# Nostrademous/dotaclient

Hardware: AMD Instinct MI355X
Metric: PPO optimizer samples/sec (whole node) + actor steps/sec, 1v1-mid LSTM policy (higher is better)
Workload: dtype fp32

## Files before the change

### dotaclient_amd/ops/csrc/gemm_tn.hip

```cpp
#include "common.h"
#include <cstdlib>

namespace {

using dca::bf16x8;
using dca::f32x4;
typedef short bf16x4v __attribute__((ext_vector_type(4)));

constexpr int BM = 128, BN = 128, BK = 64;
constexpr int kThreads = 256;
constexpr int kTileBytes = BK * 128 * 2;

__device__ __forceinline__ int lds_off(int row, int ch) {
  return 256 * row + 16 * (ch ^ (((row & 3) << 2) | ((row >> 2) & 3)));
}

__device__ __forceinline__ __amdgpu_buffer_rsrc_t uniform_rsrc(const void* p, long long bytes) {
  const unsigned long long a = (unsigned long long)p;
  const unsigned lo = __builtin_amdgcn_readfirstlane((unsigned)a);
  const unsigned hi = __builtin_amdgcn_readfirstlane((unsigned)(a >> 32));
  const int nb = (int)(bytes < 0 ? 0 : (bytes > 0x7fff0000LL ? 0x7fff0000LL : bytes));
  return __builtin_amdgcn_make_buffer_rsrc((void*)(((unsigned long long)hi << 32) | lo), (short)0,
                                           __builtin_amdgcn_readfirstlane(nb), 0x00020000);
}
constexpr int kOob = 0x7fff8000;

__device__ __forceinline__ uint4 bload16(__amdgpu_buffer_rsrc_t r, int off) {
  return __builtin_bit_cast(uint4, __builtin_amdgcn_raw_buffer_load_b128(r, off, 0, 0));
}

struct Args {
  const void* A; int lda;
  const void* B; int ldb;
  const void* B0; int split;
  float* C; int ldc;
  const int* perm;
  float* slab;
  float* colsum;
  int M, N, K, kc, splits, tiles_n, accumulate;
  int xcd_remap;
};

struct Rsrc {
  __amdgpu_buffer_rsrc_t A, B, B0;
};

__device__ __forceinline__ Rsrc make_rsrc(const Args& a, int es) {
  Rsrc r;
  r.A = uniform_rsrc(a.A, ((long long)(a.K - 1) * a.lda + a.M) * es);
  r.B = uniform_rsrc(a.B, a.K > a.split ? ((long long)(a.K - a.split - 1) * a.ldb + a.N) * es : 0);
  r.B0 = uniform_rsrc(a.B0 ? a.B0 : a.B, a.split > 0 ? ((long long)(a.split - 1) * a.ldb + a.N) * es : 0);
  return r;
}

template <bool WITH_B0>
__device__ __forceinline__ void load_stage(const Args& a, const Rsrc& R, int kbase, int kend, int m_base, int n_base,
                                           uint4 (&ra)[4], uint4 (&rb)[4]) {
  const int t = threadIdx.x, ch = t & 15;
  const int m = m_base + ch * 8, n = n_base + ch * 8;
#pragma unroll
  for (int i = 0; i < 4; ++i) {
    const int k = kbase + (t >> 4) + 16 * i;
    const bool kin = k < kend;
    ra[i] = bload16(R.A, kin && m < a.M ? (k * a.lda + m) * 2 : kOob);
    rb[i] = bload16(R.B, kin && n < a.N && k >= a.split ? ((k - a.split) * a.ldb + n) * 2 : kOob);
  }
  if (WITH_B0 && kbase < a.split) {
#pragma unroll
    for (int i = 0; i < 4; ++i) {
      const int k = kbase + (t >> 4) + 16 * i;
      const uint4 v = bload16(R.B0, k < kend && n < a.N && k < a.split ? (k * a.ldb + n) * 2 : kOob);
      rb[i] = make_uint4(rb[i].x | v.x, rb[i].y | v.y, rb[i].z | v.z, rb[i].w | v.w);
    }
  }
}

__device__ __forceinline__ void store_stage(char* As, char* Bs, const uint4 (&ra)[4], const uint4 (&rb)[4]) {
  const int t = threadIdx.x, ch = t & 15;
#pragma unroll
  for (int i = 0; i < 4; ++i) {
    const int r = (t >> 4) + 16 * i;
    *reinterpret_cast<uint4*>(As + lds_off(r, ch)) = ra[i];
    *reinterpret_cast<uint4*>(Bs + lds_off(r, ch)) = rb[i];
  }
}

__device__ __forceinline__ void colsum_acc(float (&cs)[8], const uint4 (&ra)[4]) {
#pragma unroll
  for (int i = 0; i < 4; ++i) {
    const unsigned w[4] = {ra[i].x, ra[i].y, ra[i].z, ra[i].w};
#pragma unroll
    for (int j = 0; j < 4; ++j) {
      cs[2 * j] += __uint_as_float(w[j] << 16);
      cs[2 * j + 1] += __uint_as_float(w[j] & 0xffff0000u);
    }
  }
}

struct F32Stage {
  float4 a[2][2], b[2][2];
};

template <bool WITH_B0>
__device__ __forceinline__ void load_stage_f32(const Args& a, const Rsrc& R, int kbase, int kend, int m_base,
                                               int n_base, F32Stage& r) {
  const int t = threadIdx.x, ch = t & 15;
  const int m = m_base + ch * 8, n = n_base + ch * 8;
#pragma unroll
  for (int i = 0; i < 2; ++i) {
    const int k = kbase + (t >> 4) + 16 * i;
    const bool kin = k < kend;
    const int oa = kin && m < a.M ? (k * a.lda + m) * 4 : kOob;
    const int ob = kin && n < a.N && k >= a.split ? ((k - a.split) * a.ldb + n) * 4 : kOob;
    r.a[i][0] = __builtin_bit_cast(float4, bload16(R.A, oa));
    r.a[i][1] = __builtin_bit_cast(float4, bload16(R.A, oa + 16));
    r.b[i][0] = __builtin_bit_cast(float4, bload16(R.B, ob));
    r.b[i][1] = __builtin_bit_cast(float4, bload16(R.B, ob + 16));
  }
  if (WITH_B0 && kbase < a.split) {
#pragma unroll
    for (int i = 0; i < 2; ++i) {
      const int k = kbase + (t >> 4) + 16 * i;
      const int o0 = k < kend && n < a.N && k < a.split ? (k * a.ldb + n) * 4 : kOob;
      const float4 p = __builtin_bit_cast(float4, bload16(R.B0, o0));
      const float4 q = __builtin_bit_cast(float4, bload16(R.B0, o0 + 16));
      r.b[i][0] = make_float4(r.b[i][0].x + p.x, r.b[i][0].y + p.y, r.b[i][0].z + p.z, r.b[i][0].w + p.w);
      r.b[i][1] = make_float4(r.b[i][1].x + q.x, r.b[i][1].y + q.y, r.b[i][1].z + q.z, r.b[i][1].w + q.w);
    }
  }
}

__device__ __forceinline__ unsigned pack_bf2(float x, float y) {
  return (unsigned)(unsigned short)dca::f2bf(x) | ((unsigned)(unsigned short)dca::f2bf(y) << 16);
}

__device__ __forceinline__ void split8(const float4& p, const float4& q, uint4& hi, uint4& lo) {
  const float v[8] = {p.x, p.y, p.z, p.w, q.x, q.y, q.z, q.w};
  float l[8];
#pragma unroll
  for (int j = 0; j < 8; ++j) l[j] = v[j] - dca::bf2f(dca::f2bf(v[j]));
  hi = make_uint4(pack_bf2(v[0], v[1]), pack_bf2(v[2], v[3]), pack_bf2(v[4], v[5]), pack_bf2(v[6], v[7]));
  lo = make_uint4(pack_bf2(l[0], l[1]), pack_bf2(l[2], l[3]), pack_bf2(l[4], l[5]), pack_bf2(l[6], l[7]));
}

constexpr int kImgF32 = 32 * 256;
__device__ __forceinline__ void store_stage_f32(char* S, const F32Stage& r) {
  const int t = threadIdx.x, ch = t & 15;
#pragma unroll
  for (int i = 0; i < 2; ++i) {
    const int row = (t >> 4) + 16 * i;
    uint4 hi, lo;
    split8(r.a[i][0], r.a[i][1], hi, lo);
    *reinterpret_cast<uint4*>(S + lds_off(row, ch)) = hi;
    *reinterpret_cast<uint4*>(S + kImgF32 + lds_off(row, ch)) = lo;
    split8(r.b[i][0], r.b[i][1], hi, lo);
    *reinterpret_cast<uint4*>(S + 2 * kImgF32 + lds_off(row, ch)) = hi;
    *reinterpret_cast<uint4*>(S + 3 * kImgF32 + lds_off(row, ch)) = lo;
  }
}

__device__ __forceinline__ void colsum_acc_f32(float (&cs)[8], const F32Stage& r) {
#pragma unroll
  for (int i = 0; i < 2; ++i) {
    cs[0] += r.a[i][0].x; cs[1] += r.a[i][0].y; cs[2] += r.a[i][0].z; cs[3] += r.a[i][0].w;
    cs[4] += r.a[i][1].x; cs[5] += r.a[i][1].y; cs[6] += r.a[i][1].z; cs[7] += r.a[i][1].w;
  }
}

__device__ __forceinline__ bf16x8 frag_tr(const char* img, int k0, int c0) {
  const int l = threadIdx.x & 63, g = l >> 4, i = l & 15, q = i >> 2, p = i & 3;
  const int ch = (c0 >> 3) + (p >> 1);
  const int row0 = k0 + 8 * g + q;
  typedef __attribute__((address_space(3))) bf16x4v lds_v4;
  const bf16x4v lo = __builtin_amdgcn_ds_read_tr16_b64_v4i16(
      (lds_v4*)(img + lds_off(row0, ch) + 8 * (p & 1)));
  const bf16x4v hi = __builtin_amdgcn_ds_read_tr16_b64_v4i16(
      (lds_v4*)(img + lds_off(row0 + 4, ch) + 8 * (p & 1)));
  bf16x8 f;
  f[0] = lo[0]; f[1] = lo[1]; f[2] = lo[2]; f[3] = lo[3];
  f[4] = hi[0]; f[5] = hi[1]; f[6] = hi[2]; f[7] = hi[3];
  return f;
}

__device__ __forceinline__ void tile_split(const Args& a, int& tile, int& split) {
  const int tiles = ((a.M + BM - 1) / BM) * a.tiles_n;
  const int n = gridDim.x, orig = blockIdx.x;
  const int q = n >> 3, r = n & 7, x = orig & 7;
  const int id = a.xcd_remap ? (x < r ? x * (q + 1) : r * (q + 1) + (x - r) * q) + (orig >> 3) : orig;
  tile = id % tiles;
  split = id / tiles;
}

template <bool F32>
__global__ __launch_bounds__(kThreads) void gemm_tn_kernel(Args a) {
  extern __shared__ __attribute__((aligned(16))) char smem[];
  constexpr int BKx = F32 ? 32 : BK;
#define AS(b) (smem + (b) * kTileBytes)
#define BS(b) (smem + (2 + (b)) * kTileBytes)
#define SF(b) (smem + (b) * 4 * kImgF32)
  int tile, split;
  tile_split(a, tile, split);
  const int tm = tile / a.tiles_n, tn = tile % a.tiles_n;
  const int m_base = tm * BM, n_base = tn * BN;
  const int k_lo = split * a.kc, k_hi = min(a.K, k_lo + a.kc);
  const int w = threadIdx.x >> 6, wm = w & 1, wn = w >> 1;

  f32x4 acc[4][4];
#pragma unroll
  for (int i = 0; i < 4; ++i)
#pragma unroll
    for (int j = 0; j < 4; ++j) acc[i][j] = f32x4{0.f, 0.f, 0.f, 0.f};

  uint4 ra[4], rb[4];
  F32Stage rf;
  float cs[8] = {0.f, 0.f, 0.f, 0.f, 0.f, 0.f, 0.f, 0.f};
  const bool do_cs = a.colsum != nullptr && tn == 0;
  int buf = 0;
  const Rsrc R = make_rsrc(a, F32 ? 4 : 2);
  if (k_lo < k_hi) {
    if constexpr (F32) {
      load_stage_f32<true>(a, R, k_lo, k_hi, m_base, n_base, rf);
      store_stage_f32(SF(0), rf);
      if (do_cs) colsum_acc_f32(cs, rf);
    } else {
      load_stage<true>(a, R, k_lo, k_hi, m_base, n_base, ra, rb);
      store_stage(AS(0), BS(0), ra, rb);
      if (do_cs) colsum_acc(cs, ra);
    }
  }
  __syncthreads();
  for (int kb = k_lo; kb < k_hi; kb += BKx) {
    const bool more = kb + BKx < k_hi;
    if constexpr (F32) {
      if (more) load_stage_f32<false>(a, R, kb + BKx, k_hi, m_base, n_base, rf);
      const char* S = SF(buf);
      bf16x8 fah[4], fal[4], fbh[4], fbl[4];
#pragma unroll
      for (int i = 0; i < 4; ++i) {
        fah[i] = frag_tr(S, 0, wm * 64 + i * 16);
        fal[i] = frag_tr(S + kImgF32, 0, wm * 64 + i * 16);
      }
#pragma unroll
      for (int j = 0; j < 4; ++j) {
        fbh[j] = frag_tr(S + 2 * kImgF32, 0, wn * 64 + j * 16);
        fbl[j] = frag_tr(S + 3 * kImgF32, 0, wn * 64 + j * 16);
      }
#pragma unroll
      for (int i = 0; i < 4; ++i)
#pragma unroll
        for (int j = 0; j < 4; ++j) acc[i][j] = __builtin_amdgcn_mfma_f32_16x16x32_bf16(fal[i], fbh[j], acc[i][j], 0, 0, 0);
#pragma unroll
      for (int i = 0; i < 4; ++i)
#pragma unroll
        for (int j = 0; j < 4; ++j) acc[i][j] = __builtin_amdgcn_mfma_f32_16x16x32_bf16(fah[i], fbl[j], acc[i][j], 0, 0, 0);
#pragma unroll
      for (int i = 0; i < 4; ++i)
#pragma unroll
        for (int j = 0; j < 4; ++j) acc[i][j] = __builtin_amdgcn_mfma_f32_16x16x32_bf16(fah[i], fbh[j], acc[i][j], 0, 0, 0);
      if (more) {
        store_stage_f32(SF(buf ^ 1), rf);
        if (do_cs) colsum_acc_f32(cs, rf);
      }
    } else {
      if (more) load_stage<false>(a, R, kb + BK, k_hi, m_base, n_base, ra, rb);
#pragma unroll
      for (int ks = 0; ks < BK / 32; ++ks) {
        bf16x8 fa[4], fb[4];
#pragma unroll
        for (int i = 0; i < 4; ++i) fa[i] = frag_tr(AS(buf), ks * 32, wm * 64 + i * 16);
#pragma unroll
        for (int j = 0; j < 4; ++j) fb[j] = frag_tr(BS(buf), ks * 32, wn * 64 + j * 16);
#pragma unroll
        for (int i = 0; i < 4; ++i)
#pragma unroll
          for (int j = 0; j < 4; ++j)
            acc[i][j] = __builtin_amdgcn_mfma_f32_16x16x32_bf16(fa[i], fb[j], acc[i][j], 0, 0, 0);
      }
      if (more) {
        store_stage(AS(buf ^ 1), BS(buf ^ 1), ra, rb);
        if (do_cs) colsum_acc(cs, ra);
      }
    }
    __syncthreads();
    buf ^= 1;
  }
  if (do_cs) {
    float* red = reinterpret_cast<float*>(smem);
    const int t = threadIdx.x, ch = t & 15, rg = t >> 4;
#pragma unroll
    for (int j = 0; j < 8; ++j) red[rg * 128 + ch * 8 + j] = cs[j];
    __syncthreads();
    if (t < 128) {
      float v = 0.f;
      for (int g = 0; g < 16; ++g) v += red[g * 128 + t];
      const int m = m_base + t;
      if (m < a.M) {
        if (a.splits == 1) {
          float* cp = a.colsum + (a.perm ? a.perm[m] : m);
          *cp = a.accumulate ? *cp + v : v;
        } else {
          a.slab[(size_t)a.splits * a.M * a.N + (size_t)split * a.M + m] = v;
        }
      }
    }
  }

  const int l = threadIdx.x & 63;
  if (a.splits == 1) {
#pragma unroll
    for (int i = 0; i < 4; ++i)
#pragma unroll
      for (int e = 0; e < 4; ++e) {
        const int m = m_base + wm * 64 + 16 * i + 4 * (l >> 4) + e;
        if (m >= a.M) continue;
        float* crow = a.C + (size_t)(a.perm ? a.perm[m] : m) * a.ldc;
#pragma unroll
        for (int j = 0; j < 4; ++j) {
          const int n = n_base + wn * 64 + 16 * j + (l & 15);
          if (n < a.N) crow[n] = a.accumulate ? crow[n] + acc[i][j][e] : acc[i][j][e];
        }
      }
    return;
  }
  float* slab = a.slab + (size_t)split * a.M * a.N;
#pragma unroll
  for (int i = 0; i < 4; ++i)
#pragma unroll
    for (int e = 0; e < 4; ++e) {
      const int m = m_base + wm * 64 + 16 * i + 4 * (l >> 4) + e;
      if (m >= a.M) continue;
#pragma unroll
      for (int j = 0; j < 4; ++j) {
        const int n = n_base + wn * 64 + 16 * j + (l & 15);
        if (n < a.N) slab[(size_t)m * a.N + n] = acc[i][j][e];
      }
    }
#undef AS
#undef BS
#undef SF
}

constexpr int kXP = 144;
constexpr int kXImg = 32 * kXP * 4;

struct XStage {
  float4 a[4], b[4];
};

template <bool WITH_B0>
__device__ __forceinline__ void load_stage_x(const Args& a, const Rsrc& R, int kbase, int kend, int m_base, int n_base,
                                             XStage& r) {
  const int t = threadIdx.x, c4 = 4 * (t & 31);
  const int m = m_base + c4, n = n_base + c4;
#pragma unroll
  for (int i = 0; i < 4; ++i) {
    const int k = kbase + (t >> 5) + 8 * i;
    const bool kin = k < kend;
    r.a[i] = __builtin_bit_cast(float4, bload16(R.A, kin && m < a.M ? (k * a.lda + m) * 4 : kOob));
    r.b[i] = __builtin_bit_cast(float4, bload16(R.B, kin && n < a.N && k >= a.split ? ((k - a.split) * a.ldb + n) * 4
                                                                                    : kOob));
  }
  if (WITH_B0 && kbase < a.split) {
#pragma unroll
    for (int i = 0; i < 4; ++i) {
      const int k = kbase + (t >> 5) + 8 * i;
      const float4 p = __builtin_bit_cast(float4, bload16(R.B0, k < kend && n < a.N && k < a.split ? (k * a.ldb + n) * 4
                                                                                                  : kOob));
      r.b[i] = make_float4(r.b[i].x + p.x, r.b[i].y + p.y, r.b[i].z + p.z, r.b[i].w + p.w);
    }
  }
}

__device__ __forceinline__ void store_stage_x(char* S, const XStage& r) {
  const int t = threadIdx.x, c4 = 4 * (t & 31);
#pragma unroll
  for (int i = 0; i < 4; ++i) {
    const int row = (t >> 5) + 8 * i;
    *reinterpret_cast<float4*>(S + (row * kXP + c4) * 4) = r.a[i];
    *reinterpret_cast<float4*>(S + kXImg + (row * kXP + c4) * 4) = r.b[i];
  }
}

__device__ __forceinline__ void kahan_add(float& s, float& c, float v) {
  const float y = v - c, t = s + y;
  c = (t - s) - y;
  s = t;
}
__device__ __forceinline__ void add_slab_colsum(float (&cs)[4], float (&cc)[4], const XStage& st) {
  kahan_add(cs[0], cc[0], (st.a[0].x + st.a[1].x) + (st.a[2].x + st.a[3].x));
  kahan_add(cs[1], cc[1], (st.a[0].y + st.a[1].y) + (st.a[2].y + st.a[3].y));
  kahan_add(cs[2], cc[2], (st.a[0].z + st.a[1].z) + (st.a[2].z + st.a[3].z));
  kahan_add(cs[3], cc[3], (st.a[0].w + st.a[1].w) + (st.a[2].w + st.a[3].w));
}

__global__ __launch_bounds__(kThreads, 2) void gemm_tn_exact_kernel(Args a) {
  __shared__ __attribute__((aligned(16))) char smem[4 * kXImg];
  int tile, split;
  tile_split(a, tile, split);
  const int tm = tile / a.tiles_n, tn = tile % a.tiles_n;
  const int m_base = tm * BM, n_base = tn * BN;
  const int k_lo = split * a.kc, k_hi = min(a.K, k_lo + a.kc);
  const int w = threadIdx.x >> 6, wm = w & 1, wn = w >> 1, l = threadIdx.x & 63;
  const int fr = l >> 4, fc = l & 15;

  f32x4 acc[4][4];
#pragma unroll
  for (int i = 0; i < 4; ++i)
#pragma unroll
    for (int j = 0; j < 4; ++j) acc[i][j] = f32x4{0.f, 0.f, 0.f, 0.f};
  float cs[4] = {0.f, 0.f, 0.f, 0.f}, cc[4] = {0.f, 0.f, 0.f, 0.f};
  const bool do_cs = a.colsum != nullptr && tn == 0;
  const Rsrc R = make_rsrc(a, 4);
  XStage st;
  int buf = 0;
  if (k_lo < k_hi) {
    load_stage_x<true>(a, R, k_lo, k_hi, m_base, n_base, st);
    store_stage_x(smem, st);
    if (do_cs) add_slab_colsum(cs, cc, st);
  }
  __syncthreads();
  for (int kb = k_lo; kb < k_hi; kb += 32) {
    const bool more = kb + 32 < k_hi;
    if (more) load_stage_x<false>(a, R, kb + 32, k_hi, m_base, n_base, st);
    const float* As = reinterpret_cast<const float*>(smem + buf * 2 * kXImg);
    const float* Bs = As + kXImg / 4;
    f32x4 part[4][4];
#pragma unroll
    for (int i = 0; i < 4; ++i)
#pragma unroll
      for (int j = 0; j < 4; ++j) part[i][j] = f32x4{0.f, 0.f, 0.f, 0.f};
#pragma unroll
    for (int c = 0; c < 8; ++c) {
      const int row = 4 * c + fr;
      float fa[4], fb[4];
#pragma unroll
      for (int i = 0; i < 4; ++i) fa[i] = As[row * kXP + wm * 64 + 16 * i + fc];
#pragma unroll
      for (int j = 0; j < 4; ++j) fb[j] = Bs[row * kXP + wn * 64 + 16 * j + fc];
#pragma unroll
      for (int i = 0; i < 4; ++i)
#pragma unroll
        for (int j = 0; j < 4; ++j) part[i][j] = __builtin_amdgcn_mfma_f32_16x16x4f32(fa[i], fb[j], part[i][j], 0, 0, 0);
    }
#pragma unroll
    for (int i = 0; i < 4; ++i)
#pragma unroll
      for (int j = 0; j < 4; ++j) acc[i][j] += part[i][j];
    if (more) {
      store_stage_x(smem + (buf ^ 1) * 2 * kXImg, st);
      if (do_cs) add_slab_colsum(cs, cc, st);
    }
    __syncthreads();
    buf ^= 1;
  }
  if (do_cs) {
    float* red = reinterpret_cast<float*>(smem);
    const int t = threadIdx.x, c4 = 4 * (t & 31), rg = t >> 5;
#pragma unroll
    for (int j = 0; j < 4; ++j) red[rg * 128 + c4 + j] = cs[j];
    __syncthreads();
    if (t < 128) {
      float v = 0.f;
      for (int g = 0; g < 8; ++g) v += red[g * 128 + t];
      const int m = m_base + t;
      if (m < a.M) {
        if (a.splits == 1) {
          float* cp = a.colsum + (a.perm ? a.perm[m] : m);
          *cp = a.accumulate ? *cp + v : v;
        } else {
          a.slab[(size_t)a.splits * a.M * a.N + (size_t)split * a.M + m] = v;
        }
      }
    }
  }
  float* slab = a.slab + (size_t)split * a.M * a.N;
#pragma unroll
  for (int i = 0; i < 4; ++i)
#pragma unroll
    for (int e = 0; e < 4; ++e) {
      const int m = m_base + wm * 64 + 16 * i + 4 * fr + e;
      if (m >= a.M) continue;
      if (a.splits == 1) {
        float* crow = a.C + (size_t)(a.perm ? a.perm[m] : m) * a.ldc;
#pragma unroll
        for (int j = 0; j < 4; ++j) {
          const int n = n_base + wn * 64 + 16 * j + fc;
          if (n < a.N) crow[n] = a.accumulate ? crow[n] + acc[i][j][e] : acc[i][j][e];
        }
      } else {
#pragma unroll
        for (int j = 0; j < 4; ++j) {
          const int n = n_base + wn * 64 + 16 * j + fc;
          if (n < a.N) slab[(size_t)m * a.N + n] = acc[i][j][e];
        }
      }
    }
}

__global__ __launch_bounds__(256) void gemm_tn_reduce(const float* __restrict__ slab, int splits, int M, int N,
                                                      float* __restrict__ C, int ldc, const int* __restrict__ perm,
                                                      int accumulate, float* __restrict__ colsum, int lp) {
  const int P = 1 << lp, OPB = 256 >> lp;
  const int n4 = N >> 2;
  const size_t plane4 = (size_t)M * N / 4;
  const int ph = threadIdx.x >> (8 - lp), oi = threadIdx.x & (OPB - 1);
  __shared__ f32x4 red[256];
  const int nout = M * n4;
  for (int base = blockIdx.x * OPB; base < nout; base += gridDim.x * OPB) {
    const int idx = base + oi;
    f32x4 s = {0.f, 0.f, 0.f, 0.f};
    if (idx < nout) {
      const int m = idx / n4, n = (idx % n4) * 4;
      const f32x4* src = reinterpret_cast<const f32x4*>(slab + (size_t)m * N + n);
      int sp = ph;
      for (; sp + 3 * P < splits; sp += 4 * P) {
        const f32x4 v0 = __builtin_nontemporal_load(src + (size_t)(sp + 0 * P) * plane4);
        const f32x4 v1 = __builtin_nontemporal_load(src + (size_t)(sp + 1 * P) * plane4);
        const f32x4 v2 = __builtin_nontemporal_load(src + (size_t)(sp + 2 * P) * plane4);
        const f32x4 v3 = __builtin_nontemporal_load(src + (size_t)(sp + 3 * P) * plane4);
        s += v0;
        s += v1;
        s += v2;
        s += v3;
      }
      for (; sp < splits; sp += P) s += __builtin_nontemporal_load(src + (size_t)sp * plane4);
    }
    if (P > 1) {
      red[threadIdx.x] = s;
      __syncthreads();
    }
    if (ph == 0 && idx < nout) {
      for (int k = 1; k < P; ++k) s += red[k * OPB + oi];
      const int m = idx / n4, n = (idx % n4) * 4;
      float* cp = C + (size_t)(perm ? perm[m] : m) * ldc + n;
      if (accumulate) {
        s[0] += cp[0]; s[1] += cp[1]; s[2] += cp[2]; s[3] += cp[3];
      }
      cp[0] = s[0]; cp[1] = s[1]; cp[2] = s[2]; cp[3] = s[3];
    }
    if (P > 1) __syncthreads();
  }
  if (colsum != nullptr) {
    const float* cs = slab + (size_t)splits * plane4 * 4;
    __shared__ float cred[256];
    for (int base = blockIdx.x * OPB; base < M; base += gridDim.x * OPB) {
      const int m = base + oi;
      float v = 0.f;
      if (m < M) {
        int sp = ph;
        for (; sp + 3 * P < splits; sp += 4 * P) {
          const float v0 = cs[(size_t)(sp + 0 * P) * M + m], v1 = cs[(size_t)(sp + 1 * P) * M + m];
          const float v2 = cs[(size_t)(sp + 2 * P) * M + m], v3 = cs[(size_t)(sp + 3 * P) * M + m];
          v += v0;
          v += v1;
          v += v2;
          v += v3;
        }
        for (; sp < splits; sp += P) v += cs[(size_t)sp * M + m];
      }
      cred[threadIdx.x] = v;
      __syncthreads();
      if (ph == 0 && m < M) {
        for (int k = 1; k < P; ++k) v += cred[k * OPB + oi];
        float* cp = colsum + (perm ? perm[m] : m);
        *cp = accumulate ? *cp + v : v;
      }
      __syncthreads();
    }
  }
}

}

extern "C" void dca_gemm_tn_plan(int M, int N, int K, int* splits, int* kc, int* tiles, int f32) {
  const int bk = f32 ? 32 : BK;
  const int tm = (M + BM - 1) / BM, tn = (N + BN - 1) / BN;
  const int t = tm * tn;
  const int target = f32 == 2 ? 512 : 384;
  int s = t >= target ? 1 : target / t;
  const int kmax = (K + bk - 1) / bk;
  if (s > kmax) s = kmax;
  if (s < 1) s = 1;
  int c = (K + s - 1) / s;
  c = (c + bk - 1) / bk * bk;
  s = (K + c - 1) / c;
  *splits = s;
  *kc = c;
  *tiles = t;
}

extern "C" hipError_t dca_gemm_tn(const void* A, int lda, const void* B, int ldb, const void* B0, int split_rows,
                                  float* C, int ldc, const int* perm, int accumulate, int M, int N, int K, float* slab,
                                  float* colsum, hipStream_t st, int f32) {
  if (B0 && split_rows > (f32 ? 32 : BK)) return hipErrorInvalidValue;
  int splits, kc, tiles;
  dca_gemm_tn_plan(M, N, K, &splits, &kc, &tiles, f32);
  static const int xcd_remap = [] { const char* e = getenv("DCA_GEMM_XCD"); return (e && e[0] == '0') ? 0 : 1; }();
  Args a{A, lda, B, ldb, B0 ? B0 : B, B0 ? split_rows : 0, C, ldc, perm, slab, colsum, M, N, K, kc, splits,
         (N + BN - 1) / BN, accumulate, xcd_remap};
  const dim3 grid(tiles * splits);
  if (f32 == 2) hipLaunchKernelGGL(gemm_tn_exact_kernel, grid, dim3(kThreads), 0, st, a);
  else if (f32) hipLaunchKernelGGL(gemm_tn_kernel<true>, grid, dim3(kThreads), 8 * kImgF32, st, a);
  else hipLaunchKernelGGL(gemm_tn_kernel<false>, grid, dim3(kThreads), 4 * kTileBytes, st, a);
  DCA_CHECK_LAUNCH();
  if (splits > 1) {
    int lp = 0;
    while (lp < 4 && (2 << lp) <= splits) ++lp;
    const int n = M * (N / 4), opb = 256 >> lp;
    int blocks = (n + opb - 1) / opb;
    if (blocks > 4096) blocks = 4096;
    hipLaunchKernelGGL(gemm_tn_reduce, dim3(blocks), dim3(256), 0, st, slab, splits, M, N, C, ldc, perm, accumulate,
                       colsum, lp);
    DCA_CHECK_LAUNCH();
  }
  return hipSuccess;
}
```

### dotaclient_amd/ops/gemm.py

```python
from __future__ import annotations

from typing import Optional

import torch

from . import require

def gemm_tn(a: torch.Tensor, b: torch.Tensor, out: Optional[torch.Tensor] = None, perm: Optional[torch.Tensor] = None,
            accumulate: bool = False, b0: Optional[torch.Tensor] = None,
            colsum: Optional[torch.Tensor] = None, exact: bool = False) -> torch.Tensor:
    C = require()
    M, N = a.shape[1], b.shape[1]
    if out is None:
        out = torch.empty(M if perm is None else int(perm.numel()), N, device=a.device, dtype=torch.float32)
    if b0 is not None and b0.shape[0] > _B0_MAX_ROWS:
        b, b0 = torch.cat([b0, b]), None
    C.gemm_tn(a, b, out, perm, bool(accumulate), b0, colsum, bool(exact))
    return out


_B0_MAX_ROWS = 32
```

Measured before the change: 2.207 million.

## Software-pipeline fp32 TN GEMM slab loop and pad unaligned shapes to multiples of 8

Restructures the fp32 MFMA main loop of the TN GEMM. LDS fragments are double-buffered one k-step ahead, stores of the next slab are interleaved with MFMAs through sched_group_barrier hints, the first MFMA is seeded with zero instead of a separate clear, and accumulation into acc is folded into the last k-step. The loop is split into a steady-state variant and a tail variant chosen at compile time so the 'more' checks disappear. On the Python side, shapes whose M or N is not a multiple of 8 are routed through a padded path, which adds extra allocations and copies for those calls.

Result: no change. 2.219 million (median of 6 runs) (+0.5%).

```diff
diff --git a/dotaclient_amd/ops/csrc/gemm_tn.hip b/dotaclient_amd/ops/csrc/gemm_tn.hip
--- a/dotaclient_amd/ops/csrc/gemm_tn.hip
+++ b/dotaclient_amd/ops/csrc/gemm_tn.hip
@@ -1,5 +1,6 @@
 #include "common.h"
 #include <cstdlib>
+#include <type_traits>
 
 namespace {
 
@@ -356,9 +357,9 @@
   for (int i = 0; i < 4; ++i) {
     const int k = kbase + (t >> 5) + 8 * i;
     const bool kin = k < kend;
+    const bool kb_in = WITH_B0 ? k >= a.split : true;
     r.a[i] = __builtin_bit_cast(float4, bload16(R.A, kin && m < a.M ? (k * a.lda + m) * 4 : kOob));
-    r.b[i] = __builtin_bit_cast(float4, bload16(R.B, kin && n < a.N && k >= a.split ? ((k - a.split) * a.ldb + n) * 4
-                                                                                    : kOob));
+    r.b[i] = __builtin_bit_cast(float4, bload16(R.B, kin && n < a.N && kb_in ? ((k - a.split) * a.ldb + n) * 4 : kOob));
   }
   if (WITH_B0 && kbase < a.split) {
 #pragma unroll
@@ -371,10 +372,10 @@
   }
 }
 
-__device__ __forceinline__ void store_stage_x(char* S, const XStage& r) {
+__device__ __forceinline__ void store_stage_x(char* S, const XStage& r, int i0 = 0, int n = 4) {
   const int t = threadIdx.x, c4 = 4 * (t & 31);
 #pragma unroll
-  for (int i = 0; i < 4; ++i) {
+  for (int i = i0; i < i0 + n; ++i) {
     const int row = (t >> 5) + 8 * i;
     *reinterpret_cast<float4*>(S + (row * kXP + c4) * 4) = r.a[i];
     *reinterpret_cast<float4*>(S + kXImg + (row * kXP + c4) * 4) = r.b[i];
@@ -416,42 +417,71 @@
   if (k_lo < k_hi) {
     load_stage_x<true>(a, R, k_lo, k_hi, m_base, n_base, st);
     store_stage_x(smem, st);
+  }
+  __syncthreads();
+  auto mma_slab = [&](auto more_c, int kb) {
+    constexpr bool MORE = decltype(more_c)::value;
+    if constexpr (MORE) load_stage_x<false>(a, R, kb + 32, k_hi, m_base, n_base, st);
+    const float* Af = reinterpret_cast<const float*>(smem + buf * 2 * kXImg) + fr * kXP + wm * 64 + fc;
+    const float* Bf = reinterpret_cast<const float*>(smem + buf * 2 * kXImg + kXImg) + fr * kXP + wn * 64 + fc;
+    char* Sn = smem + (buf ^ 1) * 2 * kXImg;
+    f32x4 part[4][4];
+    float fa[2][4], fb[2][4];
+    auto frags = [&](int c) {
+#pragma unroll
+      for (int i = 0; i < 4; ++i) fa[c & 1][i] = Af[4 * c * kXP + 16 * i];
+#pragma unroll
+      for (int j = 0; j < 4; ++j) fb[c & 1][j] = Bf[4 * c * kXP + 16 * j];
+    };
+    frags(0);
+    __builtin_amdgcn_sched_barrier(0);
+#pragma unroll
+    for (int c = 0; c < 8; ++c) {
+      if (c < 7) frags(c + 1);
+      if (MORE && (c == 5 || c == 6)) store_stage_x(Sn, st, 2 * (c - 5), 2);
+#pragma unroll
+      for (int i = 0; i < 4; ++i) {
+#pragma unroll
+        for (int j = 0; j < 4; ++j)
+          part[i][j] = __builtin_amdgcn_mfma_f32_16x16x4f32(fa[c & 1][i], fb[c & 1][j],
+                                                            c == 0 ? f32x4{0.f, 0.f, 0.f, 0.f} : part[i][j], 0, 0, 0);
+        if (c == 7) {
+          if (i > 0) {
+#pragma unroll
+            for (int j = 0; j < 4; ++j) acc[i - 1][j] += part[i - 1][j];
+#pragma unroll
+            for (int g = 0; g < 4; ++g) {
+              __builtin_amdgcn_sched_group_barrier(0x008, 1, 0);
+              __builtin_amdgcn_sched_group_barrier(0x002, 3, 0);
+            }
+          }
+          __builtin_amdgcn_sched_barrier(0);
+        }
+      }
+      if (MORE && (c == 5 || c == 6)) {
+#pragma unroll
+        for (int g = 0; g < 4; ++g) {
+          __builtin_amdgcn_sched_group_barrier(0x008, 4, 0);
+          __builtin_amdgcn_sched_group_barrier(0x200, 1, 0);
+        }
+      }
+      __builtin_amdgcn_sched_barrier(0);
+    }
+#pragma unroll
+    for (int j = 0; j < 4; ++j) acc[3][j] += part[3][j];
+    __builtin_amdgcn_sched_barrier(0);
+  };
+  int kb = k_lo;
+  for (; kb + 32 < k_hi; kb += 32) {
     if (do_cs) add_slab_colsum(cs, cc, st);
-  }
-  __syncthreads();
-  for (int kb = k_lo; kb < k_hi; kb += 32) {
-    const bool more = kb + 32 < k_hi;
-    if (more) load_stage_x<false>(a, R, kb + 32, k_hi, m_base, n_base, st);
-    const float* As = reinterpret_cast<const float*>(smem + buf * 2 * kXImg);
-    const float* Bs = As + kXImg / 4;
-    f32x4 part[4][4];
-#pragma unroll
-    for (int i = 0; i < 4; ++i)
-#pragma unroll
-      for (int j = 0; j < 4; ++j) part[i][j] = f32x4{0.f, 0.f, 0.f, 0.f};
-#pragma unroll
-    for (int c = 0; c < 8; ++c) {
-      const int row = 4 * c + fr;
-      float fa[4], fb[4];
-#pragma unroll
-      for (int i = 0; i < 4; ++i) fa[i] = As[row * kXP + wm * 64 + 16 * i + fc];
-#pragma unroll
-      for (int j = 0; j < 4; ++j) fb[j] = Bs[row * kXP + wn * 64 + 16 * j + fc];
-#pragma unroll
-      for (int i = 0; i < 4; ++i)
-#pragma unroll
-        for (int j = 0; j < 4; ++j) part[i][j] = __builtin_amdgcn_mfma_f32_16x16x4f32(fa[i], fb[j], part[i][j], 0, 0, 0);
-    }
-#pragma unroll
-    for (int i = 0; i < 4; ++i)
-#pragma unroll
-      for (int j = 0; j < 4; ++j) acc[i][j] += part[i][j];
-    if (more) {
-      store_stage_x(smem + (buf ^ 1) * 2 * kXImg, st);
-      if (do_cs) add_slab_colsum(cs, cc, st);
-    }
+    mma_slab(std::true_type{}, kb);
     __syncthreads();
     buf ^= 1;
+  }
+  if (kb < k_hi) {
+    if (do_cs) add_slab_colsum(cs, cc, st);
+    mma_slab(std::false_type{}, kb);
+    __syncthreads();
   }
   if (do_cs) {
     float* red = reinterpret_cast<float*>(smem);
diff --git a/dotaclient_amd/ops/gemm.py b/dotaclient_amd/ops/gemm.py
--- a/dotaclient_amd/ops/gemm.py
+++ b/dotaclient_amd/ops/gemm.py
@@ -15,8 +15,32 @@
         out = torch.empty(M if perm is None else int(perm.numel()), N, device=a.device, dtype=torch.float32)
     if b0 is not None and b0.shape[0] > _B0_MAX_ROWS:
         b, b0 = torch.cat([b0, b]), None
+    if M % 8 or N % 8:
+        return _gemm_tn_padded(C, a, b, out, perm, accumulate, b0, colsum, exact)
     C.gemm_tn(a, b, out, perm, bool(accumulate), b0, colsum, bool(exact))
     return out
 
 
 _B0_MAX_ROWS = 32
+
+
+def _gemm_tn_padded(C, a, b, out, perm, accumulate, b0, colsum, exact):
+    M, N = a.shape[1], b.shape[1]
+    Mp, Np = -(-M // 8) * 8, -(-N // 8) * 8
+    pad = torch.nn.functional.pad
+    ap, bp = pad(a, (0, Mp - M)), pad(b, (0, Np - N))
+    b0p = None if b0 is None else pad(b0, (0, Np - N))
+    rows = out.shape[0]
+    cp = out.new_zeros(rows + Mp - M, Np)
+    cp[:rows, :N] = out
+    pp = perm if perm is not None else torch.arange(M, device=a.device, dtype=torch.int32)
+    pp = torch.cat([pp, torch.arange(rows, rows + Mp - M, device=a.device, dtype=torch.int32)])
+    csp = None
+    if colsum is not None:
+        csp = colsum.new_zeros(rows + Mp - M)
+        csp[:rows] = colsum[:rows]
+    C.gemm_tn(ap, bp, cp, pp, bool(accumulate), b0p, csp, bool(exact))
+    out.copy_(cp[:rows, :N])
+    if colsum is not None:
+        colsum[:rows] = csp[:rows]
+    return out
```
